# paroj/aruco

Measured on AMD Instinct MI355X. Metric: frames/sec at 1920×1080, higher is better.
Workload: dtype u8; 1 GPU; 1920x1080 synthetic stream, ~20 markers/frame, threshold+contour+decode+LINES, no pose (config 2); distinct_frames_per_gpu=1024, markers_rendered_per_frame=20, batches_in_flight=5, build=src=b5798a92d5b7bb96 flags=[], gpu_max_hw_queues=4, parallelism=frames sharded 1 stream/GPU

## Files before the change

aruco_amd/capi.py:

```python
import ctypes as C
import os
import sys

import numpy as np

from .build import library_path

OK, E_INVALID, E_CAPACITY, E_UNSUPPORTED, E_HIP, E_OVERFLOW, E_BOARD_CONFIG = range(7)
THRES_FIXED, THRES_ADPT, THRES_CANNY = 0, 1, 2
CORNER_NONE, CORNER_HARRIS, CORNER_SUBPIX, CORNER_LINES = 0, 1, 2, 3
BOARD_NONE, BOARD_PIX, BOARD_METERS = -1, 0, 1
CALIB_USE_INTRINSIC_GUESS, CALIB_FIX_ASPECT_RATIO, CALIB_FIX_PRINCIPAL_POINT, CALIB_ZERO_TANGENT_DIST = 1, 2, 4, 8
CALIB_FIX_FOCAL_LENGTH, CALIB_FIX_K1, CALIB_FIX_K2, CALIB_FIX_K3 = 16, 32, 64, 128
CALIB_MAX_VIEW_POINTS = 512

_ERR_NAMES = {1: "ARUCOHIP_E_INVALID", 2: "ARUCOHIP_E_CAPACITY", 3: "ARUCOHIP_E_UNSUPPORTED", 4: "ARUCOHIP_E_HIP",
              5: "ARUCOHIP_E_OVERFLOW", 6: "ARUCOHIP_E_BOARD_CONFIG"}


class ArucoHipError(RuntimeError):
    def __init__(self, code, msg=""):
        super().__init__("%s (%d): %s" % (_ERR_NAMES.get(code, "error"), code, msg))
        self.code = code

# ... 19 lines not shown
                ("max_thres_planes", C.c_int32), ("triggers_per_frame", C.c_int32), ("contours_per_frame", C.c_int32),
                ("points_per_frame", C.c_int32), ("candidates_per_frame", C.c_int32), ("markers_per_frame", C.c_int32),
                ("long_walks_per_plane", C.c_int32)]


MARKER_DTYPE = np.dtype([("id", "<i4"), ("corners", "<f4", (8,)), ("ssize", "<f4"), ("has_pose", "<i4"),
                         ("pad_", "<i4"), ("rvec", "<f8", (3,)), ("tvec", "<f8", (3,))])
assert MARKER_DTYPE.itemsize == 96 and C.sizeof(Marker) == 96

SYMBOLS = [
    "arucohip_version", "arucohip_default_params", "arucohip_default_limits", "arucohip_create", "arucohip_create_ex",
    "arucohip_destroy", "arucohip_set_params", "arucohip_get_params", "arucohip_last_error_string", "arucohip_set_stream",
    "arucohip_get_stream", "arucohip_synchronize", "arucohip_detect", "arucohip_detect_batch", "arucohip_batch_status", "arucohip_batch_chunks",
    "arucohip_get_thresholded", "arucohip_get_candidates", "arucohip_threshold", "arucohip_detect_rectangles",
    "arucohip_warp", "arucohip_debug_num_contours", "arucohip_debug_contour", "arucohip_debug_candidates", "arucohip_debug_otsu",
    "arucohip_board_detect", "arucohip_calculate_extrinsics", "arucohip_stage_times", "arucohip_stage_name",
    "arucohip_enable_timing", "arucohip_kernel_times", "arucohip_threshold_exec_ms", "arucohip_kernel_name",
    "arucohip_debug_counters", "arucohip_board_detect_batch",
    "arucohip_gl_modelview", "arucohip_ogre_pose", "arucohip_gl_projection", "arucohip_ogre_projection",
    "arucohip_detect_bgr", "arucohip_detect_batch_bgr", "arucohip_bgr_to_gray", "arucohip_set_dictionary",
    "arucohip_set_decoder_callback",
    "arucohip_undistort", "arucohip_gl_modelview_n", "arucohip_gl_modelview_batch",
    "arucohip_set_pipeline_depth", "arucohip_detect_batch_submit", "arucohip_detect_batch_wait",
    "arucohip_mgpu_device_count", "arucohip_mgpu_create", "arucohip_mgpu_destroy", "arucohip_mgpu_size", "arucohip_mgpu_handle",
    "arucohip_mgpu_set_params", "arucohip_mgpu_last_error_string", "arucohip_mgpu_detect_batch", "arucohip_mgpu_detect_streams",
    "arucohip_mgpu_set_depth", "arucohip_mgpu_submit_batch", "arucohip_mgpu_submit_streams", "arucohip_mgpu_wait",
    "arucohip_compact_bytes", "arucohip_compact_markers", "arucohip_wait_event", "arucohip_detect_batch_retry_overflowed",
    "arucohip_refine_candidate_lines", "arucohip_mgpu_gather_mode", "arucohip_build_info",
    "arucohip_calibrate_camera", "arucohip_calibrate_board_batch",
    "arucohip_chromatic_board_corners", "arucohip_chromatic_create", "arucohip_chromatic_destroy", "arucohip_chromatic_train",
# ... 378 lines not shown
    def debug_candidates(self, frame=0, cap=512):
        q = np.zeros((cap, 4, 2), np.float32)
        ids = np.zeros(cap, np.int32)
        nrot = np.zeros(cap, np.int32)
        n = C.c_int(0)
        self._chk(self.L.arucohip_debug_candidates(self.h, frame, _ptr(q), _ptr(ids), _ptr(nrot), cap, C.byref(n)))
        k = n.value
        return q[:k].copy(), ids[:k].copy(), nrot[:k].copy()

    def debug_otsu(self, frame=0, cap=512):
        t = np.zeros(cap, np.int32)
        n = C.c_int(0)
        self._chk(self.L.arucohip_debug_otsu(self.h, frame, _ptr(t), cap, C.byref(n)))
        return t[:n.value].copy()

    def debug_contours(self, frame=0):
        n = C.c_int(0)
        self._chk(self.L.arucohip_debug_num_contours(self.h, frame, C.byref(n)))
        res = []
        for i in range(n.value):
            hole, sx, sy, npts = C.c_int(), C.c_int(), C.c_int(), C.c_int()
            self._chk(self.L.arucohip_debug_contour(self.h, frame, i, C.byref(hole), C.byref(sx), C.byref(sy), None, 0, C.byref(npts)))
            pts = np.zeros((npts.value, 2), np.int16)
            self._chk(self.L.arucohip_debug_contour(self.h, frame, i, C.byref(hole), C.byref(sx), C.byref(sy), _ptr(pts),
                                                    npts.value, C.byref(npts)))
            res.append({"hole": hole.value, "start": (sx.value, sy.value), "pts": pts.astype(np.int32)})
        return res

    def threshold(self, gray, method=THRES_ADPT, param1=-1.0, param2=-1.0):
        g = np.ascontiguousarray(gray, dtype=np.uint8)
# ... 407 lines not shown
```

aruco_amd/csrc/capi.hip:

```cpp
#include <hip/hip_runtime.h>

#include <algorithm>
#include <cmath>
#include <cstdio>
#include <cstring>
#include <string>
#include <vector>

#include "bits_tiles.h"
#include "handle.h"

namespace ah {
void launch_rotate_x(hipStream_t s, double* rt);
}

static EnvSettings read_env() {
    EnvSettings v;
    auto geti = [](const char* name, int dflt) {
        const char* e = getenv(name);
        return (e && *e) ? atoi(e) : dflt;
    };
    if (const char* e = getenv("ARUCOHIP_STREAMS")) v.streams = std::min(MAX_WORKERS, std::max(1, atoi(e)));
    v.graph = geti("ARUCOHIP_GRAPH", 1) != 0;
    if (const char* e = getenv("ARUCOHIP_CONTOURS")) v.contours = std::string(e) == "segments";
// ... 234 lines not shown
        if (lim->max_batch <= 2) ALLOC(b.skipn, P * (size_t)b.cap_raw * sizeof(uint4));
        ALLOC(b.stamp, P * (size_t)b.cap_raw * sizeof(unsigned long long));
        ALLOC(b.hash, P * (size_t)(b.hash_mask + 1) * sizeof(uint32_t));
    }
    ALLOC(b.gen_buf, ((P + 7) / 8 * 8) * (size_t)b.long_cap * 4 * 20);
    ALLOC(b.cdesc, P * (size_t)b.cap_cdesc * sizeof(ContourDesc));
    ALLOC(b.pool, P * (size_t)b.cap_pool * sizeof(short2));
    ALLOC(b.quads, F * b.cap_quads * sizeof(Quad));
    ALLOC(b.cands, F * b.cap_cands * sizeof(Cand));
    ALLOC(b.ncands, F * sizeof(int32_t));
    b.cap_flat = (uint32_t)std::min<size_t>(F * (size_t)std::min(b.cap_cands, 96), 65535u * 16u);
    ALLOC(b.cand_list, (size_t)b.cap_flat * sizeof(uint32_t));
    ALLOC(b.iM, (size_t)b.cap_flat * 9 * sizeof(double));
    ALLOC(b.hist, (size_t)b.cap_flat * 256 * sizeof(uint16_t));
    ALLOC(b.othr, (size_t)b.cap_flat * sizeof(int32_t));
    ALLOC(b.markers, (F * b.cap_markers + 1) * sizeof(arucohip_marker_t));
    ALLOC(b.nmarkers, F * sizeof(int32_t));
    ALLOC(b.marker_list, F * (size_t)b.cap_markers * sizeof(uint32_t));
    {
        const size_t w_cnt = (CNT_FIXED + F + 31) & ~(size_t)31, w_plane = P * TRIG_CNT_STRIDE;
        h->zero_words = w_cnt + GEN_CNT_WORDS + 3 * w_plane;
        ALLOC(h->zero_block, h->zero_words * sizeof(uint32_t));
        b.counters = h->zero_block;
        b.gen_cnt = b.counters + w_cnt;
        b.trig_cnt = b.gen_cnt + GEN_CNT_WORDS;
        b.raw_cnt = b.trig_cnt + w_plane;
        b.ring_cnt = b.raw_cnt + w_plane;
    }
    ALLOC(h->d_small_f, 8192 * sizeof(float));
    ALLOC(h->d_small_d, 64 * sizeof(double));
// ... 227 lines not shown
    return ARUCOHIP_OK;
}

static int ensure_walk_scratch(arucohip_handle* h, int nplanes, const DetectParams& dp) {
    size_t need = walk_scratch_words(nplanes, dp, h->buf.long_cap);
    if (need > 0xFFFFFFF0ull) return fail(h, ARUCOHIP_E_CAPACITY, "batch too large for 32-bit checkpoint offsets: fewer frames per batch or a smaller max size");
    HIPCHK(h, h->walk_scratch.reserve(need * sizeof(uint32_t)));
    h->buf.walk_scratch = h->walk_scratch;
    return ARUCOHIP_OK;
}

static int batch_prologue(arucohip_handle* h, const FrameGeom& g, int nframes, const DetectParams& dp) {
    int rc;
    if ((rc = ensure_walk_scratch(h, nframes * dp.nthr, dp))) return rc;
    if ((rc = ensure_bits_geometry(h, g.width, g.height))) return rc;
    HIPCHK(h, h->patches.reserve((size_t)h->buf.cap_flat * dp.warp_size * dp.warp_size));
    h->buf.patches = h->patches;
    return ARUCOHIP_OK;
}

static int user_decode_stage(arucohip_handle* h, const DetectParams& dp) {
    hipStream_t s = h->stream;
    const Buffers& b = h->buf;
    const size_t npx = (size_t)dp.warp_size * dp.warp_size;
    HIPCHK(h, h->hu_list.reserve((size_t)b.cap_flat * (sizeof(uint32_t) + sizeof(int2) + sizeof(uint32_t)) + sizeof(uint32_t)));
    uint32_t* list = h->hu_list;
    int2* dec = (int2*)(list + b.cap_flat);
    uint32_t* order = (uint32_t*)(dec + b.cap_flat);
    uint32_t* ncand_p = order + b.cap_flat;
    HIPCHK(h, hipMemcpyAsync(ncand_p, b.counters + CNT_NCAND, sizeof(uint32_t), hipMemcpyDeviceToHost, s));
    HIPCHK(h, hipStreamSynchronize(s));
    const uint32_t n = std::min(*ncand_p, b.cap_flat);
// ... 78 lines not shown
    }
    if (h->params.erode) {
        const bool on_tiles = !h->thres_bytes;
        HIPCHK(h, h->d_erode.reserve(on_tiles ? erode_tiles_tmp_bytes(g, nframes * dp.nthr) : (size_t)nframes * dp.nthr * g.width * g.height));
        if (on_tiles)
            launch_erode_tiles(s, g, nframes * dp.nthr, b, h->d_erode);
        else
            launch_erode(s, g, nframes * dp.nthr, b, h->d_erode);
    }
    MARK(K_FILTER);
    {
        const int rc_ = run_rectangles(h, s, g, nframes, dp, ev);
        if (rc_) return rc_;
    }
    MARK(K_DECODE);
    const bool fused_cells = dp.decoder == ARUCOHIP_DECODER_FIDUCIAL_5X5;
    if (RUN_STAGE(b.env, 6)) launch_decode(s, gray_dev, g, nframes, dp, b, fused_cells);
    if (dp.decoder == ARUCOHIP_DECODER_USER) {
        const int rc_ = user_decode_stage(h, dp);
        if (rc_) return rc_;
    }
    MARK(K_REFINE_LINES);
    if (RUN_STAGE(b.env, 7)) launch_refine_lines(s, g, nframes, dp, cam, b, fused_cells);
    MARK(K_REFINE_PIXELS);
    if (dp.corner_method == ARUCOHIP_CORNER_HARRIS || dp.corner_method == ARUCOHIP_CORNER_SUBPIX) {
        if (dp.locked) launch_locked_corners(s, gray_dev, g, nframes, dp, b);
        launch_refine_pixels(s, gray_dev, g, nframes, dp, b);
    }
    MARK(K_FINALIZE);
    if (RUN_STAGE(b.env, 8)) launch_finalize(s, g, nframes, dp, cam, b, h->wt_out, h->wt_cap, h->wt_n);
    MARK(K_POSE);
// ... 172 lines not shown
        const hipError_t e2 = hipStreamEndCapture(h->stream, &graph);
        const std::array<const void*, 3> captured = {gray_dev, h->buf.walk_scratch, h->buf.patches};
        if (rc != ARUCOHIP_OK || e != hipSuccess || e2 != hipSuccess || !graph || captured != addrs ||
            hipGraphInstantiate(&h->fgraph.exec, graph, nullptr, nullptr, 0) != hipSuccess) {
            (void)hipGetLastError();
            if (graph) (void)hipGraphDestroy(graph);
            h->fgraph.exec = nullptr, h->fgraph.disabled = 1;
            return ARUCOHIP_OK;
        }
        (void)hipGraphDestroy(graph);
        h->fgraph.key = key, h->fgraph.addrs = addrs, h->fgraph.thres_bytes = h->thres_bytes;
    }
    *handled = true;
    HIPCHK(h, hipGraphLaunch(h->fgraph.exec, h->stream));
    h->thres_bytes = h->fgraph.thres_bytes;
    h->last = plan_batch(h, 1, W, H, dp.nthr);
    HIPCHK(h, hipStreamSynchronize(h->stream));
    const int32_t* hdr = (const int32_t*)(h->h_markers + h->buf.cap_markers);
    h->h_n[0] = hdr[0], h->h_counters[CNT_STATUS] = (uint32_t)hdr[1];
    return collect_batch_host(h, out, cap, n_out);
}

static int detect_batch_impl(arucohip_handle* h, const uint8_t* frames, int nframes, int W, int H, size_t row_stride, size_t frame_stride,
                             int frames_on_device, int channels, const float* K, const float* dist, int ndist, float marker_size, int y_perp,
                             arucohip_marker_t* out, int cap, int32_t* n_out, int out_on_device, bool defer = false) {
    if (!h || !frames || !n_out || (cap > 0 && !out) || cap < 0) return ARUCOHIP_E_INVALID;
    int rc = check_geometry(h, nframes, W, H, row_stride, channels);
    if (rc) return rc;
    HIPCHK(h, hipSetDevice(h->device));
    DetectParams dp;
// ... 218 lines not shown
    HIPCHK(h, hipMemcpyAsync(cnt, h->buf.counters, sizeof(cnt), hipMemcpyDeviceToHost, h->stream));
    HIPCHK(h, hipMemcpyAsync(&nc, h->buf.ncands + frame, sizeof(nc), hipMemcpyDeviceToHost, h->stream));
    HIPCHK(h, hipStreamSynchronize(h->stream));
    const uint32_t nflat = std::min(cnt[CNT_NCAND], h->buf.cap_flat);
    std::vector<uint32_t> list(nflat);
    std::vector<int32_t> othr(nflat);
    if (nflat) {
        HIPCHK(h, hipMemcpyAsync(list.data(), h->buf.cand_list, nflat * sizeof(uint32_t), hipMemcpyDeviceToHost, h->stream));
        HIPCHK(h, hipMemcpyAsync(othr.data(), h->buf.othr, nflat * sizeof(int32_t), hipMemcpyDeviceToHost, h->stream));
        HIPCHK(h, hipStreamSynchronize(h->stream));
    }
    *n = std::max(nc, 0);
    for (int i = 0; i < std::min(*n, cap); i++) thr[i] = -1;
    for (uint32_t i = 0; i < nflat; i++)
        if ((int)(list[i] >> 16) == frame && (int)(list[i] & 0xFFFFu) < cap) thr[list[i] & 0xFFFFu] = othr[i];
    return *n > cap ? ARUCOHIP_E_CAPACITY : ARUCOHIP_OK;
}

int arucohip_debug_candidates(arucohip_handle* h, int frame, float* quads0, int32_t* ids, int32_t* nrot, int cap, int* n) {
    std::vector<Cand> v;
    int rc = fetch_cands(h, frame, &v);
    if (rc) return rc;
    int k = 0;
    for (auto& c : v) {
        if (k < cap) {
            for (int i = 0; i < 4; i++) quads0[k * 8 + 2 * i] = c.qx[i], quads0[k * 8 + 2 * i + 1] = c.qy[i];
            if (ids) ids[k] = c.id;
            if (nrot) nrot[k] = c.nrot;
        }
        k++;
// ... 498 lines not shown
```

aruco_amd/csrc/decode_device.h:

```cpp
#pragma once
#include "internal.h"

namespace ah {

__device__ inline bool solve8(double* A, double* b) {
    const int n = 8;
    for (int c = 0; c < n; c++) {
        int piv = c;
        double best = fabs(A[c * n + c]);
        for (int r = c + 1; r < n; r++) {
            double v = fabs(A[r * n + c]);
            if (v > best) best = v, piv = r;
        }
        if (best == 0) return false;
        if (piv != c) {
            for (int k = 0; k < n; k++) {
                double t = A[c * n + k];
                A[c * n + k] = A[piv * n + k];
                A[piv * n + k] = t;
            }
            double t = b[c];
            b[c] = b[piv];
            b[piv] = t;
        }
// ... 126 lines not shown
}

__device__ __forceinline__ int hamm_rows(const uint32_t v[5]) {
    const uint32_t words[4] = {0x01, 0x1D, 0x12, 0x0E};
    int dist = 0;
#pragma unroll
    for (int y = 0; y < 5; y++) {
        int best = 100000;
#pragma unroll
        for (int p = 0; p < 4; p++) best = min(best, __popc(v[y] ^ words[p]));
        dist += best;
    }
    return dist;
}

__device__ __forceinline__ void cells_decode_wave(const uint8_t* patch, int ws, int thr, int lane, int* id_out, int* nrot_out) {
    const int sw = ws / 7;
    const int half = (sw * sw) / 2;
    bool white = false;
    if (lane < 49) {
        const int cy = lane / 7, cx = lane - cy * 7;
        int cnt = 0;
        if (sw == 8 && (((size_t)patch | (size_t)ws) & 7) == 0) {
#pragma unroll
            for (int y = 0; y < 8; y++) {
                const uint2 w = *(const uint2*)(patch + (cy * 8 + y) * ws + cx * 8);
#pragma unroll
                for (int b = 0; b < 4; b++) cnt += (int)((w.x >> (8 * b)) & 0xFFu) > thr, cnt += (int)((w.y >> (8 * b)) & 0xFFu) > thr;
            }
        } else {
            for (int y = 0; y < sw; y++)
                for (int x = 0; x < sw; x++) cnt += patch[(cy * sw + y) * ws + cx * sw + x] > thr;
        }
        white = cnt > half;
    }
    const unsigned long long m = __ballot(white);
    int id = -1, nrot = 0;
    if (lane == 0) {
        unsigned long long border = 0x7Full | (0x7Full << 42);
#pragma unroll
        for (int y = 1; y < 6; y++) border |= (1ull << (7 * y)) | (1ull << (7 * y + 6));
        if ((m & border) == 0) {
            uint32_t cur[5], best[5];
#pragma unroll
            for (int y = 0; y < 5; y++) cur[y] = (uint32_t)(m >> (7 * (y + 1) + 1)) & 31u, best[y] = cur[y];
            int min_dist = hamm_rows(cur);
#pragma unroll
            for (int r = 1; r < 4; r++) {
                uint32_t nxt[5];
#pragma unroll
                for (int i = 0; i < 5; i++) {
                    nxt[i] = 0;
#pragma unroll
                    for (int j = 0; j < 5; j++) nxt[i] |= ((cur[4 - j] >> i) & 1u) << j;
                }
#pragma unroll
                for (int i = 0; i < 5; i++) cur[i] = nxt[i];
                const int dd = hamm_rows(cur);
                if (dd < min_dist) {
                    min_dist = dd, nrot = r;
#pragma unroll
                    for (int i = 0; i < 5; i++) best[i] = cur[i];
                }
            }
            if (min_dist == 0) {
                id = 0;
#pragma unroll
                for (int y = 0; y < 5; y++) id |= (int)((((best[y] >> 1) & 1u) << 1) | ((best[y] >> 3) & 1u)) << (2 * (4 - y));
            }
        }
    }
    *id_out = id, *nrot_out = nrot;
}

}
```

aruco_amd/csrc/handle.h:

```cpp
#pragma once
#include <hip/hip_runtime.h>

#include <algorithm>
#include <array>
#include <cstdio>
#include <string>
#include <vector>

#include "internal.h"

using namespace ah;

enum { K_THRESHOLD = 0, K_FILTER, K_WALKERS, K_WALKERS_LONG, K_CONTOUR_QUADS, K_FRAME_CANDS, K_DECODE, K_REFINE_LINES, K_REFINE_PIXELS, K_FINALIZE, K_POSE, K_COUNT };
constexpr int TSETS = 32;

template <typename T>
struct Mem {
    T* p = nullptr;
    size_t bytes = 0;
    bool pinned = false;
    explicit Mem(bool pinned_ = false) : pinned(pinned_) {}
    Mem(Mem&& o) noexcept : p(o.p), bytes(o.bytes), pinned(o.pinned) { o.p = nullptr, o.bytes = 0; }
    ~Mem() { (void)release(); }
    operator T*() const { return p; }
// ... 43 lines not shown
struct Dictionary {
    int n = 0, count = 0, tau0 = 0;
    float rate = 1.f;
    std::vector<uint64_t> codes;
};

struct arucohip_handle {
    int device = 0;
    hipStream_t own_stream = nullptr, stream = nullptr;
    arucohip_params_t params;
    arucohip_limits_t lim;
    Buffers buf{};
    std::vector<Mem<void>> held;
    Mem<uint32_t> walk_scratch;
    Mem<uint8_t> patches;
    Mem<uint8_t> d_gray;
    Mem<uint8_t> d_bgr;
    arucohip_marker_t* wt_out = nullptr;
    int32_t* wt_n = nullptr;
    int wt_cap = 0;
    Mem<uint8_t> d_erode;
    Mem<uint64_t> d_canny;
    Mem<short2> d_umap_xy;
    Mem<uint16_t> d_umap_f;
    int umap_w = 0, umap_h = 0, umap_nd = -1;
    float umap_K[9] = {}, umap_d[8] = {};
    Mem<uint8_t> d_undist;
    Dictionary hrm;
    Mem<uint64_t> d_hrm;
    arucohip_decoder_fn decoder_fn = nullptr;
// ... 74 lines not shown
```

aruco_amd/csrc/internal.h:

```cpp
#pragma once
#include <hip/hip_runtime.h>
#include <stdint.h>

#include "../../include/arucohip.h"

namespace ah {

constexpr int WAVE = 64;
constexpr int TRIG_CNT_STRIDE = 32;
constexpr int TC_CDESC = 2;
constexpr int TC_POOL = 3;
constexpr int TC_STATUS = 5;
constexpr int TC_SNAP = 4;
constexpr int WALK_BLOCKS = 16;


enum Counter {
    CNT_NMARK = 0,
    CNT_UNUSED1 = 1,
    CNT_UNUSED2 = 2,
    CNT_STATUS = 3,
    CNT_NCAND = 5,
    CNT_FIXED = 8
};
// ... 112 lines not shown
    int thr_stamp_on;
    uint32_t* walk_scratch;
    uint4* node;
    uint4* skipn;
    unsigned long long* stamp;
    uint32_t* hash;
    uint32_t hash_mask;
    Quad* quads;
    Cand* cands;
    int32_t* ncands;
    uint32_t* cand_list;
    double* iM;
    uint16_t* hist;
    int32_t* othr;
    uint8_t* patches;
    uint32_t cap_flat;
    arucohip_marker_t* markers;
    int32_t* nmarkers;
    uint32_t* marker_list;
    uint32_t* counters;
    uint32_t cap_raw, cap_trig;
    uint32_t long_cap;
    int seg_mode, grid_mask;
    uint32_t cap_cdesc, cap_pool;
    int cap_quads, cap_cands, cap_markers;
};

#ifndef LBP_PRIO
#define LBP_PRIO 3
#endif
// ... 15 lines not shown
void launch_erode_tiles(hipStream_t s, const FrameGeom& g, int nplanes, const Buffers& b, uint8_t* tmp);
void launch_tile_bitmap(hipStream_t s, const FrameGeom& g, int nplanes, const Buffers& b);
void launch_binary_planes(hipStream_t s, const uint8_t* thres_in, const FrameGeom& g, int nframes, const Buffers& b);
void launch_start_candidates(hipStream_t s, const FrameGeom& g, int nplanes, const Buffers& b, int min_contour = 0);
struct WalkFork {
    hipStream_t side;
    hipEvent_t forked, joined;
    hipEvent_t after_first;
};
bool launch_walkers(hipStream_t s, const WalkFork& fk, const FrameGeom& g, int nplanes, const DetectParams& p, const Buffers& b);
size_t walk_scratch_words(int nplanes, const DetectParams& p, uint32_t long_cap);
constexpr size_t GEN_CNT_WORDS = 2 * 32 * 32 * 8;
void launch_segments(hipStream_t s, const FrameGeom& g, int nplanes, const DetectParams& p, const Buffers& b);
void launch_contour_quads(hipStream_t s, const FrameGeom& g, int nframes, const DetectParams& p, const Buffers& b, int pass = 0);
void launch_frame_candidates(hipStream_t s, const FrameGeom& g, int nframes, const DetectParams& p, const Buffers& b);
void launch_decode(hipStream_t s, const uint8_t* gray, const FrameGeom& g, int nframes, const DetectParams& p, const Buffers& b, bool fused_cells = false);
void launch_set_decoded(hipStream_t s, const Buffers& b, uint32_t n, const int2* id_nrot_dev);
void launch_refine_lines(hipStream_t s, const FrameGeom& g, int nframes, const DetectParams& p, const CamModel& cam, const Buffers& b, bool fused_cells = false);
void launch_locked_corners(hipStream_t s, const uint8_t* gray, const FrameGeom& g, int nframes, const DetectParams& p, const Buffers& b);
void launch_refine_pixels(hipStream_t s, const uint8_t* gray, const FrameGeom& g, int nframes, const DetectParams& p, const Buffers& b);
void launch_finalize(hipStream_t s, const FrameGeom& g, int nframes, const DetectParams& p, const CamModel& cam, const Buffers& b, arucohip_marker_t* out = nullptr,
                     int out_cap = 0, int32_t* n_out = nullptr);
void launch_pose(hipStream_t s, int nframes, const CamModel& cam, const Buffers& b);
void launch_warp_only(hipStream_t s, const uint8_t* gray, const FrameGeom& g, const float* quad_dev, int size, uint8_t* dst_dev);
void launch_pnp_points(hipStream_t s, const float* obj, const float* img, int npts, const CamModel& cam, double* rt_out, int* ok_out);
void launch_project_points(hipStream_t s, const float* obj, int npts, const double* rt, const CamModel& cam, float* img_out);
void launch_gl_modelview(hipStream_t s, int nframes, int cap, const Buffers& b, double* out_dev);
void launch_marker_pose(hipStream_t s, arucohip_marker_t* markers, int n, const CamModel& cam);
void launch_board_pose(hipStream_t s, int nframes, const Buffers& b, const int32_t* ids, const float* obj, int nboard, int info_type,
                       float marker_size, float repj_thres, const CamModel& cam, arucohip_board_t* out, float* prob);
// ... 101 lines not shown
```

aruco_amd/csrc/k_decode.hip:

```cpp
#include <float.h>
#include <limits.h>

#include <algorithm>

#include "internal.h"
#include "decode_device.h"

namespace ah {

__device__ static void inverse_homography(const float* quad, int size, double* A, double* b, double* iM) {
    const float d = (float)(size - 1);
    const float dst[8] = {0, 0, d, 0, d, d, 0, d};
    perspective_transform_solve(quad, dst, A, b);
    double m[9];
    for (int i = 0; i < 8; i++) m[i] = b[i];
    m[8] = 1.0;
    double det = m[0] * (m[4] * m[8] - m[5] * m[7]) - m[1] * (m[3] * m[8] - m[5] * m[6]) + m[2] * (m[3] * m[7] - m[4] * m[6]);
    det = det != 0 ? 1. / det : 0;
    iM[0] = (m[4] * m[8] - m[5] * m[7]) * det;
    iM[1] = (m[2] * m[7] - m[1] * m[8]) * det;
    iM[2] = (m[1] * m[5] - m[2] * m[4]) * det;
    iM[3] = (m[5] * m[6] - m[3] * m[8]) * det;
    iM[4] = (m[0] * m[8] - m[2] * m[6]) * det;
    iM[5] = (m[2] * m[3] - m[0] * m[5]) * det;
// ... 16 lines not shown
}

struct DecodeArgs {
    const uint8_t* gray;
    size_t row_stride, frame_stride;
    int width, height, ws;
    Cand* cands;
    int cap_cands;
    const uint32_t* cand_list;
    const uint32_t* counters;
    uint32_t cap_flat;
    double* iM;
    uint16_t* hist;
    int32_t* othr;
    uint8_t* patches;
};


#ifndef HCOPIES_N
#define HCOPIES_N 32
#endif
constexpr int HCOPIES = HCOPIES_N, HPITCH = 65;
constexpr int HWCOPIES = HCOPIES / 4, HWPITCH = 257;
constexpr int HLANES = WAVE / HCOPIES;
#ifndef GQ_N
#define GQ_N 7
#endif
#ifndef XCD_RUN_N
#define XCD_RUN_N 48
#endif
// ... 13 lines not shown
    if (!sure) {
        const double Wd = Wq != 0 ? 1. / Wq : 0;
        fX = fmax((double)INT_MIN, fmin((double)INT_MAX, nx * Wd));
        fY = fmax((double)INT_MIN, fmin((double)INT_MAX, ny * Wd));
    }
    const int X = __double2int_rn(fX), Y = __double2int_rn(fY);
    uint8_t v = 0;
    if (FAST) {
        if ((int)((uint32_t)X < (uint32_t)W) & (int)((uint32_t)Y < (uint32_t)H)) v = src[(uint32_t)Y * (uint32_t)row_stride + (uint32_t)X];
    } else {
        if (inside && X >= 0 && X < W && Y >= 0 && Y < H) v = src[(size_t)Y * row_stride + X];
    }
    return v;
}

template <int WS, int ROWS>
__device__ __forceinline__ void warp_hist_candidate(const DecodeArgs& a, const uint32_t idx, uint32_t* hist, const double* siM, const int lane) {
    const uint32_t e = a.cand_list[idx];
    const uint8_t* src = a.gray + (size_t)(e >> 16) * a.frame_stride;
    const int W = a.width, H = a.height;
    const int ws = WS ? WS : a.ws, npx = ws * ws;
    const bool bytes = HLANES * ((ws + 7) / 8) * ((ws + 7) / 8) < 256;
    uint8_t* patch = a.patches + (size_t)idx * npx;
    uint32_t* myhist = bytes ? hist + (lane / HLANES) * HPITCH : hist + (lane & (HWCOPIES - 1)) * HWPITCH;
    const double m0 = siM[0], m1 = siM[1], m2 = siM[2], m3 = siM[3], m4 = siM[4], m5 = siM[5], m6 = siM[6], m7 = siM[7], m8 = siM[8];
    const int bxl = lane & 7, byl = lane >> 3;
    uint32_t psum = 0;
    if (WS == 8 * GQ) {
        double ax[GQ], bx[GQ], cx[GQ];
#pragma unroll
        for (int q = 0; q < GQ; q++) {
            const int x = q * 8 + bxl;
            ax[q] = m0 * x, bx[q] = m3 * x, cx[q] = m6 * x;
        }
        uint8_t* prow = patch + byl * WS + bxl;
        for (int BY0 = 0; BY0 < GQ; BY0 += ROWS) {
            uint8_t v[ROWS][GQ];
#pragma unroll
            for (int rr = 0; rr < ROWS; rr++) {
                const int BY = min(BY0 + rr, GQ - 1);
                const int y = BY * 8 + byl;
                const double X0 = m1 * y + m2, Y0 = m4 * y + m5, W0 = m7 * y + m8;
#pragma unroll
                for (int q = 0; q < GQ; q++) v[rr][q] = warp_gather<true>(src, a.row_stride, W, H, X0, Y0, W0, ax[q], bx[q], cx[q], true);
            }
#pragma unroll
            for (int rr = 0; rr < ROWS; rr++) {
                const int BY = BY0 + rr;
                if (BY < GQ) {
#pragma unroll
                    for (int q = 0; q < GQ; q++) {
                        prow[BY * 8 * WS + q * 8] = v[rr][q];
                        psum += v[rr][q];
                        atomicAdd(&myhist[v[rr][q] >> 2], 1u << (8 * (v[rr][q] & 3)));
                    }
                }
            }
        }
    } else {
        const int nb = (ws + 7) >> 3, nblocks = nb * nb;
        for (int b0 = 0; b0 < nblocks; b0 += GQ) {
            uint8_t v[GQ];
            int px[GQ], py[GQ];
#pragma unroll
            for (int q = 0; q < GQ; q++) {
                const int bi = b0 + q, BY = bi / nb, BX = bi - BY * nb;
                const int x = BX * 8 + bxl, y = BY * 8 + byl;
                px[q] = x, py[q] = (bi < nblocks && x < ws && y < ws) ? y : -1;
                v[q] = warp_gather<false>(src, a.row_stride, W, H, m1 * y + m2, m4 * y + m5, m7 * y + m8, m0 * x, m3 * x, m6 * x, py[q] >= 0);
            }
// ... 15 lines not shown
    if (bytes) {
        uint32_t even = 0, odd = 0;
#pragma unroll
        for (int c = 0; c < HCOPIES; c++) {
            const uint32_t w = hist[c * HPITCH + lane];
            even += w & 0x00FF00FFu, odd += (w >> 8) & 0x00FF00FFu;
        }
        hsum[0] = even & 0xFFFFu, hsum[2] = even >> 16, hsum[1] = odd & 0xFFFFu, hsum[3] = odd >> 16;
    } else {
#pragma unroll
        for (int c = 0; c < HWCOPIES; c++)
#pragma unroll
            for (int q = 0; q < 4; q++) hsum[q] += hist[c * HWPITCH + 4 * lane + q];
    }
    ((uint2*)(a.hist + (size_t)idx * 256))[lane] = make_uint2(hsum[0] | (hsum[1] << 16), hsum[2] | (hsum[3] << 16));
#pragma unroll
    for (int o = 32; o > 0; o >>= 1) psum += (uint32_t)__shfl_xor((int)psum, o, 64);
    if (lane == 0) a.othr[idx] = (int32_t)psum;
}

#ifndef WARP_WAVES_N
#define WARP_WAVES_N 2
#endif
template <int ROWS>
__global__ __launch_bounds__(64) __attribute__((amdgpu_waves_per_eu(WARP_WAVES_N, WARP_WAVES_N))) void warp_hist_kernel(DecodeArgs a) {
    throughput_bound_priority();
    __shared__ uint32_t hist[HCOPIES * HPITCH];
    __shared__ double siM[9];
    const uint32_t n = min(a.counters[CNT_NCAND], a.cap_flat);
    const int lane = threadIdx.x;
    const uint32_t nslots = ((n + 8 * XCD_RUN - 1) / (8 * XCD_RUN)) * (8 * XCD_RUN);
    for (uint32_t b = blockIdx.x; b < nslots; b += gridDim.x) {
        uint32_t idx = b;
        if (XCD_RUN > 1) {
            const uint32_t xcd = b & 7u, r = b >> 3;
            idx = ((r / XCD_RUN) * 8u + xcd) * XCD_RUN + (r % XCD_RUN);
        }
        if (idx >= n) continue;
        __syncthreads();
        for (int i = lane; i < HCOPIES * HPITCH; i += WAVE) hist[i] = 0;
        if (lane < 9) siM[lane] = a.iM[(size_t)idx * 9 + lane];
        __syncthreads();
        if (a.ws == 8 * GQ && a.row_stride * (size_t)a.height < ((size_t)1 << 32))
            warp_hist_candidate<8 * GQ, ROWS>(a, idx, hist, siM, lane);
        else
            warp_hist_candidate<0, 1>(a, idx, hist, siM, lane);
    }
}

constexpr int OTSU_PITCH = 66;
constexpr int OTSU_BINS = 64;
__global__ __launch_bounds__(64) void otsu_kernel(DecodeArgs a) {
    latency_bound_priority();
    __shared__ uint16_t sh[OTSU_BINS * OTSU_PITCH];
    const uint32_t n = min(a.counters[CNT_NCAND], a.cap_flat);
    const uint32_t base = blockIdx.x * 64;
    if (base >= n) return;
    const int lane = threadIdx.x;
    const int cnt = (int)min(64u, n - base);
    const uint32_t idx = base + min(lane, cnt - 1);
    const int npx = a.ws * a.ws;
    const double scale = 1. / npx;
    const double mu = (double)(uint32_t)a.othr[idx] * scale;
    double mu1 = 0, q1 = 0, max_sigma = 0, max_val = 0;
    constexpr int DW = OTSU_BINS / 2;
    constexpr int CPL = 64 / DW;
// ... 50 lines not shown
#pragma unroll
                for (int j = 0; j < G; j++) {
                    if ((skip >> j) & 1u) continue;
                    const int i = stage * OTSU_BINS + g0 + j;
                    const double q2 = 1. - q1v[j];
                    const double mu2 = (mu - q1v[j] * m1v[j]) / q2;
                    const double sigma = q1v[j] * q2 * (m1v[j] - mu2) * (m1v[j] - mu2);
                    if (sigma > max_sigma) {
                        max_sigma = sigma;
                        max_val = i;
                    }
                }
            }
        }
    }
    if (lane < cnt) a.othr[idx] = (int)max_val;
}

__global__ __launch_bounds__(64) void cells_decode_kernel(DecodeArgs a) {
    latency_bound_priority();
    const uint32_t n = min(a.counters[CNT_NCAND], a.cap_flat);
    const int lane = threadIdx.x;
    for (uint32_t idx = blockIdx.x; idx < n; idx += gridDim.x) {
        const uint32_t e = a.cand_list[idx];
        Cand* cand = a.cands + (size_t)(e >> 16) * a.cap_cands + (e & 0xFFFFu);
        int id, nrot;
        cells_decode_wave(a.patches + (size_t)idx * a.ws * a.ws, a.ws, a.othr[idx], lane, &id, &nrot);
        if (lane == 0) cand->id = id, cand->nrot = nrot;
    }
}

// ... 40 lines not shown
                if (hd < dm) dm = hd, rm = (uint32_t)r;
            }
            if (dm < (uint32_t)nn) best = min(best, (dm << 16) | ((uint32_t)i << 2) | rm);
        }
#pragma unroll
        for (int o = 32; o > 0; o >>= 1) best = min(best, (uint32_t)__shfl_xor((int)best, o, 64));
        if (lane == 0) {
            int id = -1, nrot = 0;
            if (best != 0xFFFFFFFFu && (best >> 16) <= d.correction) id = (int)((best >> 2) & 0x3FFFu), nrot = (int)(best & 3u);
            cand->id = id;
            cand->nrot = nrot;
        }
    }
}

void launch_decode(hipStream_t s, const uint8_t* gray, const FrameGeom& g, int nframes, const DetectParams& p, const Buffers& b, bool fused_cells) {
    DecodeArgs a;
    a.gray = gray, a.row_stride = g.row_stride, a.frame_stride = g.frame_stride, a.width = g.width, a.height = g.height;
    a.ws = p.warp_size, a.cands = b.cands, a.cap_cands = b.cap_cands;
    a.cand_list = b.cand_list, a.counters = b.counters, a.cap_flat = b.cap_flat, a.iM = b.iM, a.hist = b.hist, a.othr = b.othr, a.patches = b.patches;
    const int lane_blocks = (int)((b.cap_flat + 63) / 64);
    const int wave_blocks = (int)std::min<uint32_t>(b.cap_flat, (uint32_t)nframes * 48u);
    const int warp_blocks = nframes <= 2 ? (int)std::min<uint32_t>(b.cap_flat, 8u * XCD_RUN) : wave_blocks;
    if (nframes <= 2)
        hipLaunchKernelGGL(warp_hist_kernel<2>, dim3(warp_blocks), dim3(64), 0, s, a);
    else
        hipLaunchKernelGGL(warp_hist_kernel<1>, dim3(warp_blocks), dim3(64), 0, s, a);
    if (p.decoder == ARUCOHIP_DECODER_USER) return;
    hipLaunchKernelGGL(otsu_kernel, dim3(lane_blocks), dim3(64), 0, s, a);
    if (p.decoder == 1) {
        HrmArgs d{p.hrm_n, p.hrm_count, p.hrm_correction, p.hrm_codes};
        hipLaunchKernelGGL(hrm_decode_kernel, dim3(wave_blocks), dim3(64), 0, s, a, d);
    } else if (!fused_cells) {
        hipLaunchKernelGGL(cells_decode_kernel, dim3(wave_blocks), dim3(64), 0, s, a);
    }
}

__global__ void set_decoded_kernel(Cand* cands, int cap_cands, const uint32_t* cand_list, uint32_t n, const int2* dec) {
    const uint32_t i = blockIdx.x * blockDim.x + threadIdx.x;
    if (i >= n) return;
    const uint32_t e = cand_list[i];
    Cand* c = cands + (size_t)(e >> 16) * cap_cands + (e & 0xFFFFu);
    c->id = dec[i].x, c->nrot = dec[i].y;
}
// ... 20 lines not shown
```

include/arucohip.h:

```cpp
#ifndef ARUCOHIP_H
#define ARUCOHIP_H

#include <stddef.h>
#include <stdint.h>

#ifdef __cplusplus
extern "C" {
#endif

#define ARUCOHIP_VERSION 100

enum {
    ARUCOHIP_OK = 0,
    ARUCOHIP_E_INVALID = 1,
    ARUCOHIP_E_CAPACITY = 2,
    ARUCOHIP_E_UNSUPPORTED = 3,
    ARUCOHIP_E_HIP = 4,
    ARUCOHIP_E_OVERFLOW = 5,
    ARUCOHIP_E_BOARD_CONFIG = 6
};

enum { ARUCOHIP_THRES_FIXED = 0, ARUCOHIP_THRES_ADPT = 1, ARUCOHIP_THRES_CANNY = 2 };
enum { ARUCOHIP_CORNER_NONE = 0, ARUCOHIP_CORNER_HARRIS = 1, ARUCOHIP_CORNER_SUBPIX = 2, ARUCOHIP_CORNER_LINES = 3 };
enum { ARUCOHIP_BOARD_NONE = -1, ARUCOHIP_BOARD_PIX = 0, ARUCOHIP_BOARD_METERS = 1 };
// ... 112 lines not shown
int arucohip_threshold(arucohip_handle* h, int method, const uint8_t* gray, int width, int height, size_t row_stride,
                       double param1, double param2, uint8_t* dst);
int arucohip_detect_rectangles(arucohip_handle* h, const uint8_t* thres, int width, int height, size_t row_stride,
                               float* quads, int cap, int* n);
int arucohip_warp(arucohip_handle* h, const uint8_t* gray, int width, int height, size_t row_stride, const float quad[8],
                  int size, uint8_t* dst);

int arucohip_refine_candidate_lines(arucohip_handle* h, const int32_t* contour_xy, int npoints, float corners[8], const float* K,
                                    const float* dist, int ndist);

int arucohip_debug_num_contours(arucohip_handle* h, int frame, int* n);
int arucohip_debug_contour(arucohip_handle* h, int frame, int index, int* is_hole, int* start_x, int* start_y, int16_t* xy,
                           int cap_points, int* n_points);
int arucohip_debug_candidates(arucohip_handle* h, int frame, float* quads0, int32_t* ids, int32_t* nrot, int cap, int* n);
int arucohip_debug_otsu(arucohip_handle* h, int frame, int32_t* thr, int cap, int* n);

int arucohip_debug_counters(arucohip_handle* h, uint32_t* out8);

int arucohip_debug_hrm_stream(arucohip_handle* h, uint32_t seed, uint64_t offset, int count, uint32_t* out);
int arucohip_debug_hrm_counters(arucohip_handle* h, int32_t out[4]);

int arucohip_board_detect(arucohip_handle* h, const arucohip_marker_t* markers, int n, const int32_t* ids, const float* obj,
                          int nboard, int info_type, const float* K, const float* dist, int ndist, float marker_size,
                          float repj_err_thres, int y_perpendicular, arucohip_marker_t* out_markers, arucohip_board_t* out,
                          float* prob);

int arucohip_board_detect_batch(arucohip_handle* h, int nframes, const int32_t* ids, const float* obj, int nboard, int info_type,
                                const float* K, const float* dist, int ndist, float marker_size, float repj_err_thres,
                                int y_perpendicular, arucohip_board_t* out, float* prob);

// ... 96 lines not shown
```

Baseline: 380,800 frames/s.

## Compute cell medians during warp-histogram gather and decode inside Otsu kernel

For batched 5x5 fiducial decoding with 56-pixel warps, the warp-histogram kernel now computes each 8x8 cell's median with a ballot-based bitwise rank search instead of writing the full warped patch to memory. The Otsu kernel then thresholds the 49 stored medians, decodes the marker word and writes id/rotation directly, so the separate cells-decode kernel and the patch buffer are no longer needed on this path. This cuts patch write/read traffic and one kernel launch, at the cost of eight ballot reductions per gathered pixel group, and raises waves-per-EU to 4 for this variant. A debug API for reading the cells is added as well.

```diff
diff --git a/aruco_amd/capi.py b/aruco_amd/capi.py
--- a/aruco_amd/capi.py
+++ b/aruco_amd/capi.py
@@ -57,6 +57,7 @@
     "arucohip_get_stream", "arucohip_synchronize", "arucohip_detect", "arucohip_detect_batch", "arucohip_batch_status", "arucohip_batch_chunks",
     "arucohip_get_thresholded", "arucohip_get_candidates", "arucohip_threshold", "arucohip_detect_rectangles",
     "arucohip_warp", "arucohip_debug_num_contours", "arucohip_debug_contour", "arucohip_debug_candidates", "arucohip_debug_otsu",
+    "arucohip_debug_cells",
     "arucohip_board_detect", "arucohip_calculate_extrinsics", "arucohip_stage_times", "arucohip_stage_name",
     "arucohip_enable_timing", "arucohip_kernel_times", "arucohip_threshold_exec_ms", "arucohip_kernel_name",
     "arucohip_debug_counters", "arucohip_board_detect_batch",
@@ -465,6 +466,12 @@
         self._chk(self.L.arucohip_debug_otsu(self.h, frame, _ptr(t), cap, C.byref(n)))
         return t[:n.value].copy()
 
+    def debug_cells(self, frame=0, cap=512):
+        c = np.zeros((cap, 7, 7), np.uint8)
+        n = C.c_int(0)
+        self._chk(self.L.arucohip_debug_cells(self.h, frame, _ptr(c), cap, C.byref(n)))
+        return c[:n.value].copy()
+
     def debug_contours(self, frame=0):
         n = C.c_int(0)
         self._chk(self.L.arucohip_debug_num_contours(self.h, frame, C.byref(n)))
diff --git a/aruco_amd/csrc/capi.hip b/aruco_amd/csrc/capi.hip
--- a/aruco_amd/csrc/capi.hip
+++ b/aruco_amd/csrc/capi.hip
@@ -272,6 +272,7 @@
     ALLOC(b.iM, (size_t)b.cap_flat * 9 * sizeof(double));
     ALLOC(b.hist, (size_t)b.cap_flat * 256 * sizeof(uint16_t));
     ALLOC(b.othr, (size_t)b.cap_flat * sizeof(int32_t));
+    ALLOC(b.cells, (size_t)b.cap_flat * 64);
     ALLOC(b.markers, (F * b.cap_markers + 1) * sizeof(arucohip_marker_t));
     ALLOC(b.nmarkers, F * sizeof(int32_t));
     ALLOC(b.marker_list, F * (size_t)b.cap_markers * sizeof(uint32_t));
@@ -529,8 +530,10 @@
     int rc;
     if ((rc = ensure_walk_scratch(h, nframes * dp.nthr, dp))) return rc;
     if ((rc = ensure_bits_geometry(h, g.width, g.height))) return rc;
-    HIPCHK(h, h->patches.reserve((size_t)h->buf.cap_flat * dp.warp_size * dp.warp_size));
-    h->buf.patches = h->patches;
+    if (!decode_from_cells(g, nframes, dp)) {
+        HIPCHK(h, h->patches.reserve((size_t)h->buf.cap_flat * dp.warp_size * dp.warp_size));
+        h->buf.patches = h->patches;
+    }
     return ARUCOHIP_OK;
 }
 
@@ -639,7 +642,8 @@
         if (rc_) return rc_;
     }
     MARK(K_DECODE);
-    const bool fused_cells = dp.decoder == ARUCOHIP_DECODER_FIDUCIAL_5X5;
+    h->cells_valid = decode_from_cells(g, nframes, dp);
+    const bool fused_cells = dp.decoder == ARUCOHIP_DECODER_FIDUCIAL_5X5 && !h->cells_valid;
     if (RUN_STAGE(b.env, 6)) launch_decode(s, gray_dev, g, nframes, dp, b, fused_cells);
     if (dp.decoder == ARUCOHIP_DECODER_USER) {
         const int rc_ = user_decode_stage(h, dp);
@@ -842,6 +846,7 @@
     *handled = true;
     HIPCHK(h, hipGraphLaunch(h->fgraph.exec, h->stream));
     h->thres_bytes = h->fgraph.thres_bytes;
+    h->cells_valid = false;
     h->last = plan_batch(h, 1, W, H, dp.nthr);
     HIPCHK(h, hipStreamSynchronize(h->stream));
     const int32_t* hdr = (const int32_t*)(h->h_markers + h->buf.cap_markers);
@@ -1090,6 +1095,35 @@
     for (int i = 0; i < std::min(*n, cap); i++) thr[i] = -1;
     for (uint32_t i = 0; i < nflat; i++)
         if ((int)(list[i] >> 16) == frame && (int)(list[i] & 0xFFFFu) < cap) thr[list[i] & 0xFFFFu] = othr[i];
+    return *n > cap ? ARUCOHIP_E_CAPACITY : ARUCOHIP_OK;
+}
+
+int arucohip_debug_cells(arucohip_handle* h0, int frame, uint8_t* cells49, int cap, int* n) {
+    if (!h0 || !cells49 || !n) return ARUCOHIP_E_INVALID;
+    arucohip_handle* h = h0->last.holder(frame, &frame);
+    if (!h) return ARUCOHIP_E_INVALID;
+    if (!h->cells_valid) return fail(h, ARUCOHIP_E_INVALID, "the last batch did not decode from cell medians");
+    HIPCHK(h, hipSetDevice(h->device));
+    uint32_t cnt[CNT_FIXED];
+    int32_t nc = 0;
+    HIPCHK(h, hipMemcpyAsync(cnt, h->buf.counters, sizeof(cnt), hipMemcpyDeviceToHost, h->stream));
+    HIPCHK(h, hipMemcpyAsync(&nc, h->buf.ncands + frame, sizeof(nc), hipMemcpyDeviceToHost, h->stream));
+    HIPCHK(h, hipStreamSynchronize(h->stream));
+    const uint32_t nflat = std::min(cnt[CNT_NCAND], h->buf.cap_flat);
+    std::vector<uint32_t> list(nflat);
+    std::vector<uint8_t> cells((size_t)nflat * 64);
+    if (nflat) {
+        HIPCHK(h, hipMemcpyAsync(list.data(), h->buf.cand_list, nflat * sizeof(uint32_t), hipMemcpyDeviceToHost, h->stream));
+        HIPCHK(h, hipMemcpyAsync(cells.data(), h->buf.cells, cells.size(), hipMemcpyDeviceToHost, h->stream));
+        HIPCHK(h, hipStreamSynchronize(h->stream));
+    }
+    *n = std::max(nc, 0);
+    for (uint32_t i = 0; i < nflat; i++) {
+        const int ci = (int)(list[i] & 0xFFFFu);
+        if ((int)(list[i] >> 16) != frame || ci >= cap) continue;
+        for (int cy = 0; cy < 7; cy++)
+            for (int cx = 0; cx < 7; cx++) cells49[(size_t)ci * 49 + cy * 7 + cx] = cells[(size_t)i * 64 + cy * 8 + cx];
+    }
     return *n > cap ? ARUCOHIP_E_CAPACITY : ARUCOHIP_OK;
 }
 
diff --git a/aruco_amd/csrc/decode_device.h b/aruco_amd/csrc/decode_device.h
--- a/aruco_amd/csrc/decode_device.h
+++ b/aruco_amd/csrc/decode_device.h
@@ -164,9 +164,49 @@
     return dist;
 }
 
+__device__ __forceinline__ void fiducial_decode_word(unsigned long long m, int* id_out, int* nrot_out) {
+    int id = -1, nrot = 0;
+    unsigned long long border = 0x7Full | (0x7Full << 42);
+#pragma unroll
+    for (int y = 1; y < 6; y++) border |= (1ull << (7 * y)) | (1ull << (7 * y + 6));
+    if ((m & border) == 0) {
+        uint32_t cur[5], best[5];
+#pragma unroll
+        for (int y = 0; y < 5; y++) cur[y] = (uint32_t)(m >> (7 * (y + 1) + 1)) & 31u, best[y] = cur[y];
+        int min_dist = hamm_rows(cur);
+#pragma unroll
+        for (int r = 1; r < 4; r++) {
+            uint32_t nxt[5];
+#pragma unroll
+            for (int i = 0; i < 5; i++) {
+                nxt[i] = 0;
+#pragma unroll
+                for (int j = 0; j < 5; j++) nxt[i] |= ((cur[4 - j] >> i) & 1u) << j;
+            }
+#pragma unroll
+            for (int i = 0; i < 5; i++) cur[i] = nxt[i];
+            const int dd = hamm_rows(cur);
+            if (dd < min_dist) {
+                min_dist = dd, nrot = r;
+#pragma unroll
+                for (int i = 0; i < 5; i++) best[i] = cur[i];
+            }
+        }
+        if (min_dist == 0) {
+            id = 0;
+#pragma unroll
+            for (int y = 0; y < 5; y++) id |= (int)((((best[y] >> 1) & 1u) << 1) | ((best[y] >> 3) & 1u)) << (2 * (4 - y));
+        }
+    }
+    *id_out = id, *nrot_out = nrot;
+}
+
+constexpr int CELLS_PITCH = 8;
+constexpr int cell_vote_rank(int sw) { return (sw * sw) / 2 + 1; }
+
 __device__ __forceinline__ void cells_decode_wave(const uint8_t* patch, int ws, int thr, int lane, int* id_out, int* nrot_out) {
     const int sw = ws / 7;
-    const int half = (sw * sw) / 2;
+    const int half = cell_vote_rank(sw) - 1;
     bool white = false;
     if (lane < 49) {
         const int cy = lane / 7, cx = lane - cy * 7;
@@ -186,40 +226,7 @@
     }
     const unsigned long long m = __ballot(white);
     int id = -1, nrot = 0;
-    if (lane == 0) {
-        unsigned long long border = 0x7Full | (0x7Full << 42);
-#pragma unroll
-        for (int y = 1; y < 6; y++) border |= (1ull << (7 * y)) | (1ull << (7 * y + 6));
-        if ((m & border) == 0) {
-            uint32_t cur[5], best[5];
-#pragma unroll
-            for (int y = 0; y < 5; y++) cur[y] = (uint32_t)(m >> (7 * (y + 1) + 1)) & 31u, best[y] = cur[y];
-            int min_dist = hamm_rows(cur);
-#pragma unroll
-            for (int r = 1; r < 4; r++) {
-                uint32_t nxt[5];
-#pragma unroll
-                for (int i = 0; i < 5; i++) {
-                    nxt[i] = 0;
-#pragma unroll
-                    for (int j = 0; j < 5; j++) nxt[i] |= ((cur[4 - j] >> i) & 1u) << j;
-                }
-#pragma unroll
-                for (int i = 0; i < 5; i++) cur[i] = nxt[i];
-                const int dd = hamm_rows(cur);
-                if (dd < min_dist) {
-                    min_dist = dd, nrot = r;
-#pragma unroll
-                    for (int i = 0; i < 5; i++) best[i] = cur[i];
-                }
-            }
-            if (min_dist == 0) {
-                id = 0;
-#pragma unroll
-                for (int y = 0; y < 5; y++) id |= (int)((((best[y] >> 1) & 1u) << 1) | ((best[y] >> 3) & 1u)) << (2 * (4 - y));
-            }
-        }
-    }
+    if (lane == 0) fiducial_decode_word(m, &id, &nrot);
     *id_out = id, *nrot_out = nrot;
 }
 
diff --git a/aruco_amd/csrc/handle.h b/aruco_amd/csrc/handle.h
--- a/aruco_amd/csrc/handle.h
+++ b/aruco_amd/csrc/handle.h
@@ -81,6 +81,7 @@
     std::vector<Mem<void>> held;
     Mem<uint32_t> walk_scratch;
     Mem<uint8_t> patches;
+    bool cells_valid = false;
     Mem<uint8_t> d_gray;
     Mem<uint8_t> d_bgr;
     arucohip_marker_t* wt_out = nullptr;
diff --git a/aruco_amd/csrc/internal.h b/aruco_amd/csrc/internal.h
--- a/aruco_amd/csrc/internal.h
+++ b/aruco_amd/csrc/internal.h
@@ -150,6 +150,7 @@
     uint16_t* hist;
     int32_t* othr;
     uint8_t* patches;
+    uint8_t* cells;
     uint32_t cap_flat;
     arucohip_marker_t* markers;
     int32_t* nmarkers;
@@ -195,6 +196,7 @@
 void launch_segments(hipStream_t s, const FrameGeom& g, int nplanes, const DetectParams& p, const Buffers& b);
 void launch_contour_quads(hipStream_t s, const FrameGeom& g, int nframes, const DetectParams& p, const Buffers& b, int pass = 0);
 void launch_frame_candidates(hipStream_t s, const FrameGeom& g, int nframes, const DetectParams& p, const Buffers& b);
+bool decode_from_cells(const FrameGeom& g, int nframes, const DetectParams& p);
 void launch_decode(hipStream_t s, const uint8_t* gray, const FrameGeom& g, int nframes, const DetectParams& p, const Buffers& b, bool fused_cells = false);
 void launch_set_decoded(hipStream_t s, const Buffers& b, uint32_t n, const int2* id_nrot_dev);
 void launch_refine_lines(hipStream_t s, const FrameGeom& g, int nframes, const DetectParams& p, const CamModel& cam, const Buffers& b, bool fused_cells = false);
diff --git a/aruco_amd/csrc/k_decode.hip b/aruco_amd/csrc/k_decode.hip
--- a/aruco_amd/csrc/k_decode.hip
+++ b/aruco_amd/csrc/k_decode.hip
@@ -54,6 +54,7 @@
     uint16_t* hist;
     int32_t* othr;
     uint8_t* patches;
+    uint8_t* cells;
 };
 
 
@@ -97,14 +98,16 @@
     return v;
 }
 
-template <int WS, int ROWS>
+template <int WS, int ROWS, bool CELLS>
 __device__ __forceinline__ void warp_hist_candidate(const DecodeArgs& a, const uint32_t idx, uint32_t* hist, const double* siM, const int lane) {
     const uint32_t e = a.cand_list[idx];
     const uint8_t* src = a.gray + (size_t)(e >> 16) * a.frame_stride;
     const int W = a.width, H = a.height;
     const int ws = WS ? WS : a.ws, npx = ws * ws;
     const bool bytes = HLANES * ((ws + 7) / 8) * ((ws + 7) / 8) < 256;
-    uint8_t* patch = a.patches + (size_t)idx * npx;
+    static_assert(!CELLS || (WS == 8 * GQ && WS / 7 == 8 && GQ <= CELLS_PITCH), "a wave-gather must be a cell of the 7 x 7 grid");
+    uint8_t* patch = CELLS ? nullptr : a.patches + (size_t)idx * npx;
+    uint32_t mycell = 0;
     uint32_t* myhist = bytes ? hist + (lane / HLANES) * HPITCH : hist + (lane & (HWCOPIES - 1)) * HWPITCH;
     const double m0 = siM[0], m1 = siM[1], m2 = siM[2], m3 = siM[3], m4 = siM[4], m5 = siM[5], m6 = siM[6], m7 = siM[7], m8 = siM[8];
     const int bxl = lane & 7, byl = lane >> 3;
@@ -131,12 +134,24 @@
             for (int rr = 0; rr < ROWS; rr++) {
                 const int BY = BY0 + rr;
                 if (BY < GQ) {
+                    uint32_t rowcells[2] = {0, 0};
 #pragma unroll
                     for (int q = 0; q < GQ; q++) {
-                        prow[BY * 8 * WS + q * 8] = v[rr][q];
+                        if (CELLS) {
+                            uint32_t t = 0;
+#pragma unroll
+                            for (int bit = 7; bit >= 0; bit--) {
+                                const uint32_t c = t | (1u << bit);
+                                if (__popcll(__ballot((uint32_t)v[rr][q] >= c)) >= cell_vote_rank(8)) t = c;
+                            }
+                            rowcells[q >> 2] |= t << (8 * (q & 3));
+                        } else {
+                            prow[BY * 8 * WS + q * 8] = v[rr][q];
+                        }
                         psum += v[rr][q];
                         atomicAdd(&myhist[v[rr][q] >> 2], 1u << (8 * (v[rr][q] & 3)));
                     }
+                    if (CELLS && byl == BY) mycell = ((bxl < 4 ? rowcells[0] : rowcells[1]) >> (8 * (bxl & 3))) & 0xFFu;
                 }
             }
         }
@@ -182,6 +197,7 @@
             for (int q = 0; q < 4; q++) hsum[q] += hist[c * HWPITCH + 4 * lane + q];
     }
     ((uint2*)(a.hist + (size_t)idx * 256))[lane] = make_uint2(hsum[0] | (hsum[1] << 16), hsum[2] | (hsum[3] << 16));
+    if (CELLS) a.cells[(size_t)idx * 64 + lane] = (uint8_t)mycell;
 #pragma unroll
     for (int o = 32; o > 0; o >>= 1) psum += (uint32_t)__shfl_xor((int)psum, o, 64);
     if (lane == 0) a.othr[idx] = (int32_t)psum;
@@ -190,8 +206,9 @@
 #ifndef WARP_WAVES_N
 #define WARP_WAVES_N 2
 #endif
-template <int ROWS>
-__global__ __launch_bounds__(64) __attribute__((amdgpu_waves_per_eu(WARP_WAVES_N, WARP_WAVES_N))) void warp_hist_kernel(DecodeArgs a) {
+constexpr int WARP_WAVES_CELLS = 4;
+template <int ROWS, bool CELLS>
+__global__ __launch_bounds__(64) __attribute__((amdgpu_waves_per_eu(CELLS ? WARP_WAVES_CELLS : WARP_WAVES_N, CELLS ? WARP_WAVES_CELLS : WARP_WAVES_N))) void warp_hist_kernel(DecodeArgs a) {
     throughput_bound_priority();
     __shared__ uint32_t hist[HCOPIES * HPITCH];
     __shared__ double siM[9];
@@ -209,15 +226,18 @@
         for (int i = lane; i < HCOPIES * HPITCH; i += WAVE) hist[i] = 0;
         if (lane < 9) siM[lane] = a.iM[(size_t)idx * 9 + lane];
         __syncthreads();
-        if (a.ws == 8 * GQ && a.row_stride * (size_t)a.height < ((size_t)1 << 32))
-            warp_hist_candidate<8 * GQ, ROWS>(a, idx, hist, siM, lane);
+        if (CELLS)
+            warp_hist_candidate<8 * GQ, ROWS, true>(a, idx, hist, siM, lane);
+        else if (a.ws == 8 * GQ && a.row_stride * (size_t)a.height < ((size_t)1 << 32))
+            warp_hist_candidate<8 * GQ, ROWS, false>(a, idx, hist, siM, lane);
         else
-            warp_hist_candidate<0, 1>(a, idx, hist, siM, lane);
+            warp_hist_candidate<0, 1, false>(a, idx, hist, siM, lane);
     }
 }
 
 constexpr int OTSU_PITCH = 66;
 constexpr int OTSU_BINS = 64;
+template <bool DECODE>
 __global__ __launch_bounds__(64) void otsu_kernel(DecodeArgs a) {
     latency_bound_priority();
     __shared__ uint16_t sh[OTSU_BINS * OTSU_PITCH];
@@ -298,7 +318,28 @@
             }
         }
     }
-    if (lane < cnt) a.othr[idx] = (int)max_val;
+    if (lane < cnt) {
+        const int thr = (int)max_val;
+        a.othr[idx] = thr;
+        if (DECODE) {
+            const uint2* row = (const uint2*)(a.cells + (size_t)idx * 64);
+            unsigned long long m = 0;
+#pragma unroll
+            for (int cy = 0; cy < 7; cy++) {
+                const uint2 w = row[cy];
+#pragma unroll
+                for (int cx = 0; cx < 7; cx++) {
+                    const int px = (int)(((cx < 4 ? w.x : w.y) >> (8 * (cx & 3))) & 0xFFu);
+                    m |= (unsigned long long)(px > thr) << (cy * 7 + cx);
+                }
+            }
+            int id, nrot;
+            fiducial_decode_word(m, &id, &nrot);
+            const uint32_t e = a.cand_list[idx];
+            Cand* cand = a.cands + (size_t)(e >> 16) * a.cap_cands + (e & 0xFFFFu);
+            cand->id = id, cand->nrot = nrot;
+        }
+    }
 }
 
 __global__ __launch_bounds__(64) void cells_decode_kernel(DecodeArgs a) {
@@ -369,20 +410,27 @@
     }
 }
 
+bool decode_from_cells(const FrameGeom& g, int nframes, const DetectParams& p) {
+    return nframes > 2 && p.decoder == ARUCOHIP_DECODER_FIDUCIAL_5X5 && p.warp_size == 8 * GQ && g.row_stride * (size_t)g.height < ((size_t)1 << 32);
+}
+
 void launch_decode(hipStream_t s, const uint8_t* gray, const FrameGeom& g, int nframes, const DetectParams& p, const Buffers& b, bool fused_cells) {
     DecodeArgs a;
     a.gray = gray, a.row_stride = g.row_stride, a.frame_stride = g.frame_stride, a.width = g.width, a.height = g.height;
     a.ws = p.warp_size, a.cands = b.cands, a.cap_cands = b.cap_cands;
-    a.cand_list = b.cand_list, a.counters = b.counters, a.cap_flat = b.cap_flat, a.iM = b.iM, a.hist = b.hist, a.othr = b.othr, a.patches = b.patches;
+    a.cand_list = b.cand_list, a.counters = b.counters, a.cap_flat = b.cap_flat, a.iM = b.iM, a.hist = b.hist, a.othr = b.othr, a.patches = b.patches, a.cells = b.cells;
+    const bool cells = decode_from_cells(g, nframes, p);
     const int lane_blocks = (int)((b.cap_flat + 63) / 64);
     const int wave_blocks = (int)std::min<uint32_t>(b.cap_flat, (uint32_t)nframes * 48u);
     const int warp_blocks = nframes <= 2 ? (int)std::min<uint32_t>(b.cap_flat, 8u * XCD_RUN) : wave_blocks;
-    if (nframes <= 2)
-        hipLaunchKernelGGL(warp_hist_kernel<2>, dim3(warp_blocks), dim3(64), 0, s, a);
-    else
-        hipLaunchKernelGGL(warp_hist_kernel<1>, dim3(warp_blocks), dim3(64), 0, s, a);
+    auto* const warp_hist = cells ? warp_hist_kernel<1, true> : nframes <= 2 ? warp_hist_kernel<2, false> : warp_hist_kernel<1, false>;
+    hipLaunchKernelGGL(warp_hist, dim3(warp_blocks), dim3(64), 0, s, a);
     if (p.decoder == ARUCOHIP_DECODER_USER) return;
-    hipLaunchKernelGGL(otsu_kernel, dim3(lane_blocks), dim3(64), 0, s, a);
+    if (cells) {
+        hipLaunchKernelGGL(otsu_kernel<true>, dim3(lane_blocks), dim3(64), 0, s, a);
+        return;
+    }
+    hipLaunchKernelGGL(otsu_kernel<false>, dim3(lane_blocks), dim3(64), 0, s, a);
     if (p.decoder == 1) {
         HrmArgs d{p.hrm_n, p.hrm_count, p.hrm_correction, p.hrm_codes};
         hipLaunchKernelGGL(hrm_decode_kernel, dim3(wave_blocks), dim3(64), 0, s, a, d);
diff --git a/include/arucohip.h b/include/arucohip.h
--- a/include/arucohip.h
+++ b/include/arucohip.h
@@ -150,6 +150,7 @@
                            int cap_points, int* n_points);
 int arucohip_debug_candidates(arucohip_handle* h, int frame, float* quads0, int32_t* ids, int32_t* nrot, int cap, int* n);
 int arucohip_debug_otsu(arucohip_handle* h, int frame, int32_t* thr, int cap, int* n);
+int arucohip_debug_cells(arucohip_handle* h, int frame, uint8_t* cells49, int cap, int* n);
 
 int arucohip_debug_counters(arucohip_handle* h, uint32_t* out8);
 
```

Measured after the change: 387,300 frames/s (median of 6 runs). +1.7%, better.
